# fpthink/3D-WSIS

Measured on AMD Instinct MI355X. Metric: scenes/sec fwd+bwd ScanNet 2cm (~150k voxels) @1/8 GPU; HBM GB/s vs roofline, higher is better.
Workload: dtype f32; 1 GPU; C2: 1 synthetic ScanNet-shaped scene on 1 GPU, 2 cm voxels, fwd+bwd+AdamW step (SubMConv3d UNet 32..160 + ECC GNN + edge affinity + MultiTaskLoss); per-batch segment CSRs / edge graph and all rulebooks are rebuilt inside every step; active_voxels=153685, points=199790, superpoints=2289, edges=20054, scenes_per_gpu=1, global_batch=1, parallelism=scene-sharded dp1

## Files before the change

3d-wsis_amd/csrc/gru.hip:

```cpp
#include <algorithm>
#include <cstdlib>

#include "common.h"

using namespace wsis;

namespace {

constexpr int GC = 32;
constexpr int G3 = 96;
constexpr int GRU_WAVES = 4;
constexpr int GRU_WF = 8;
constexpr int GRU_P = 2 * G3 * GC + GC * GC + 2 * G3 + GC;

__device__ __forceinline__ float wsum(float v) {
#pragma unroll
  for (int off = 32; off >= 1; off >>= 1) v += __shfl_xor(v, off, 64);
  return v;
}
__device__ __forceinline__ float sigm(float v) { return 1.0f / (1.0f + expf(-v)); }

struct GruLds {
  float WigT[GC][GC + 1];
  float WihT[GC][G3 + 1];
  float WhhT[GC][G3 + 1];
  float Wih[G3][GC];
  float Whh[G3][GC];
  float Wig[GC][GC];
  float row[GRU_WF][4][G3];
};

template <int NT>
__device__ __forceinline__ void gru_load_weights(GruLds& L, const float* Wig, const float* Wih, const float* Whh,
// ... 119 lines not shown
    for (int u = 0; u < U; ++u) acc += v[u];
  }
  for (; j < end; j += 2) acc += m[(int64_t)perm[j] * GC + c];
  acc += __shfl_xor(acc, 32, 64);
  const int cnt = end - beg;
  return acc / (float)(cnt > 0 ? cnt : 1);
}

template <bool MEAN>
__global__ __launch_bounds__(64 * GRU_WF) void gru_fwd_kernel(
    const float* __restrict__ x, const int32_t* __restrict__ perm, const int32_t* __restrict__ off,
    float* __restrict__ x_out, const float* __restrict__ h, const float* __restrict__ Wig,
    const float* __restrict__ big, const float* __restrict__ Wih, const float* __restrict__ Whh,
    const float* __restrict__ bih, const float* __restrict__ bhh, float* __restrict__ hy, int64_t S) {
  extern __shared__ __attribute__((aligned(16))) unsigned char smem[];
  GruLds& L = *reinterpret_cast<GruLds*>(smem);
  gru_load_weights<64 * GRU_WF>(L, Wig, Wih, Whh, false);
  __syncthreads();
  const int lane = threadIdx.x & 63, wave = threadIdx.x >> 6;
  const int64_t nw = (int64_t)gridDim.x * GRU_WF;
  for (int64_t row = (int64_t)blockIdx.x * GRU_WF + wave; row < S; row += nw) {
    float xv;
    if (MEAN) {
      xv = gru_seg_mean(x, perm, off, row, lane);
      if (lane < 32) x_out[row * GC + lane] = xv;
    } else {
      xv = x[row * GC + (lane & 31)];
    }
    const GruRow R = gru_row_fwd(L, wave, lane, xv, h, big, bih, bhh, row);
    if (lane < 32) hy[row * GC + lane] = R.hy;
  }
}

__global__ __launch_bounds__(64 * GRU_WAVES) void gru_bwd_kernel(
    const float* __restrict__ x, const float* __restrict__ h, const float* __restrict__ Wig,
    const float* __restrict__ big, const float* __restrict__ Wih, const float* __restrict__ Whh,
    const float* __restrict__ bih, const float* __restrict__ bhh, const float* __restrict__ dhy,
    const float* __restrict__ dhy2, int64_t dhy2_pitch,
    float* __restrict__ dx, float* __restrict__ dh, float* __restrict__ partial, int64_t S) {
  extern __shared__ __attribute__((aligned(16))) unsigned char smem[];
  GruLds& L = *reinterpret_cast<GruLds*>(smem);
  gru_load_weights<64 * GRU_WAVES>(L, Wig, Wih, Whh, true);
  __syncthreads();
  const int lane = threadIdx.x & 63, wave = threadIdx.x >> 6;
  const int c = lane & 31, hi = lane >> 5;
  const bool two = lane < 32;
  const int64_t nw = (int64_t)gridDim.x * GRU_WAVES;
  float aWih[48], aWhh[48], aWig[16];
#pragma unroll
  for (int t = 0; t < 48; ++t) aWih[t] = aWhh[t] = 0.f;
#pragma unroll
  for (int t = 0; t < 16; ++t) aWig[t] = 0.f;
  float abih1 = 0.f, abih2 = 0.f, abhh1 = 0.f, abhh2 = 0.f, abig = 0.f;
  float* hrow = L.row[wave][0];
  float* xrow = L.row[wave][1];
  float* dgi = L.row[wave][2];
  float* dgh = L.row[wave][3];
  for (int64_t row = (int64_t)blockIdx.x * GRU_WAVES + wave; row < S; row += nw) {
    const GruRow R = gru_row_fwd(L, wave, lane, x[row * GC + c], h, big, bih, bhh, row);
    float g = dhy ? dhy[row * GC + c] : 0.0f;
    if (dhy2) g = dhy ? g + dhy2[row * dhy2_pitch + c] : dhy2[row * dhy2_pitch + c];
    const float dn = g * (1.0f - R.z);
    const float dz = g * (R.h - R.n);
    float dhc = g * R.z;
    const float dn_pre = dn * (1.0f - R.n * R.n);
    const float ghn = R.gh2 + bhh[64 + c];
    const float dr = dn_pre * ghn;
    const float dz_pre = dz * R.z * (1.0f - R.z);
    const float dr_pre = dr * R.r * (1.0f - R.r);
    const float dz_pre_up = __shfl(dz_pre, c, 64);
    const float y_i1 = two ? dr_pre : dz_pre_up;
    const float y_h1 = y_i1;
    const float y_i2 = dn_pre;
    const float y_h2 = dn_pre * R.r;
    abih1 += y_i1;
    abhh1 += y_h1;
    if (two) {
      abih2 += y_i2;
      abhh2 += y_h2;
    }
    const float inv96 = 1.0f / (float)G3;
    const float m1i = wsum(y_i1 + (two ? y_i2 : 0.f)) * inv96;
    const float m2i = wsum(y_i1 * R.gi1 + (two ? y_i2 * R.gi2 : 0.f)) * inv96;
    const float m1h = wsum(y_h1 + (two ? y_h2 : 0.f)) * inv96;
    const float m2h = wsum(y_h1 * R.gh1 + (two ? y_h2 * R.gh2 : 0.f)) * inv96;
    const float dgi1 = (y_i1 - m1i - R.gi1 * m2i) * R.sig_i;
    const float dgi2 = (y_i2 - m1i - R.gi2 * m2i) * R.sig_i;
    const float dgh1 = (y_h1 - m1h - R.gh1 * m2h) * R.sig_h;
    const float dgh2 = (y_h2 - m1h - R.gh2 * m2h) * R.sig_h;
    dgi[lane] = dgi1;
    dgh[lane] = dgh1;
    if (two) {
      dgi[64 + lane] = dgi2;
      dgh[64 + lane] = dgh2;
    }
    float dxin = 0.f, dhh = 0.f;
#pragma unroll
    for (int t = 0; t < 48; ++t) {
      const int o = hi + 2 * t;
      const float gi_o = dgi[o], gh_o = dgh[o];
      dxin += L.Wih[o][c] * gi_o;
      dhh += L.Whh[o][c] * gh_o;
      aWih[t] += gi_o * xrow[c];
      aWhh[t] += gh_o * hrow[c];
    }
    dxin += __shfl_xor(dxin, 32, 64);
    dhh += __shfl_xor(dhh, 32, 64);
    const float dxc = dxin * R.gin;
    const float dgin = dxin * R.x;
    const float dgpre = dgin * R.gin * (1.0f - R.gin);
    abig += dgpre;
    float* dgp = dgi;
    if (lane < 32) dgp[c] = dgpre;
    float dhg = 0.f;
#pragma unroll
    for (int t = 0; t < 16; ++t) {
      const int cc = hi + 2 * t;
      const float gp = dgp[cc];
      dhg += L.Wig[cc][c] * gp;
      aWig[t] += gp * hrow[c];
    }
    dhg += __shfl_xor(dhg, 32, 64);
    dhc += dhh + dhg;
    if (lane < 32) {
      dx[row * GC + c] = dxc;
      dh[row * GC + c] = dhc;
    }
  }
  __syncthreads();
  float* const mine = reinterpret_cast<float*>(smem) + wave * GRU_P;
#pragma unroll
  for (int t = 0; t < 48; ++t) {
    const int o = hi + 2 * t;
    mine[o * GC + c] = aWih[t];
    mine[G3 * GC + o * GC + c] = aWhh[t];
  }
#pragma unroll
  for (int t = 0; t < 16; ++t) mine[2 * G3 * GC + (hi + 2 * t) * GC + c] = aWig[t];
  {
    float* pb = mine + 2 * G3 * GC + GC * GC;
    pb[lane] = abih1;
    pb[G3 + lane] = abhh1;
    if (two) {
      pb[64 + lane] = abih2;
      pb[G3 + 64 + lane] = abhh2;
      pb[2 * G3 + lane] = abig;
    }
  }
  __syncthreads();
  const float* const s0 = reinterpret_cast<const float*>(smem);
  float* p = partial + (int64_t)blockIdx.x * GRU_P;
  for (int f = threadIdx.x; f < GRU_P; f += blockDim.x) {
    float v = s0[f];
#pragma unroll
    for (int w = 1; w < GRU_WAVES; ++w) v += s0[w * GRU_P + f];
    p[f] = v;
  }
}

constexpr int RED_OUT = 32;
constexpr int RED_LANES = 8;

__global__ __launch_bounds__(RED_OUT * RED_LANES) void gru_reduce_kernel(
    const float* __restrict__ partial, int nslab, float* __restrict__ dWih, float* __restrict__ dWhh,
    float* __restrict__ dWig, float* __restrict__ dbih, float* __restrict__ dbhh, float* __restrict__ dbig) {
  __shared__ float part[RED_LANES][RED_OUT];
  const int ox = threadIdx.x % RED_OUT, sy = threadIdx.x / RED_OUT;
  const int i = blockIdx.x * RED_OUT + ox;
  float s = 0.f;
  if (i < GRU_P) {
    int k = sy;
    for (; k + 15 * RED_LANES < nslab; k += 16 * RED_LANES) {
      float t[16];
#pragma unroll
      for (int j = 0; j < 16; ++j) t[j] = partial[(int64_t)(k + j * RED_LANES) * GRU_P + i];
#pragma unroll
      for (int j = 0; j < 16; ++j) s += t[j];
    }
    for (; k < nslab; k += RED_LANES) s += partial[(int64_t)k * GRU_P + i];
  }
  part[sy][ox] = s;
  __syncthreads();
  if (sy != 0 || i >= GRU_P) return;
#pragma unroll
  for (int y = 1; y < RED_LANES; ++y) s += part[y][ox];
  if (i < G3 * GC)
    dWih[i] = s;
  else if (i < 2 * G3 * GC)
    dWhh[i - G3 * GC] = s;
  else if (i < 2 * G3 * GC + GC * GC)
    dWig[i - 2 * G3 * GC] = s;
  else if (i < 2 * G3 * GC + GC * GC + G3)
    dbih[i - (2 * G3 * GC + GC * GC)] = s;
  else if (i < 2 * G3 * GC + GC * GC + 2 * G3)
    dbhh[i - (2 * G3 * GC + GC * GC + G3)] = s;
  else
    dbig[i - (2 * G3 * GC + GC * GC + 2 * G3)] = s;
}

int gru_blocks(int64_t S, int waves = GRU_WAVES, int rows_per_wave = 3) {
  const char* e = getenv("WSIS_GRU_ROWS");
  if (e && waves == GRU_WAVES && atoi(e) > 0) rows_per_wave = atoi(e);
  int64_t b = ceil_div(S, waves * rows_per_wave);
  if (b < 1) b = 1;
  if (b > 256) b = 256;
  return (int)b;
}

}

extern "C" {

int64_t wsis_gru_cell_workspace_bytes(int64_t S) {
  if (S < 0) return -1;
  return (int64_t)gru_blocks(S) * GRU_P * (int64_t)sizeof(float) + 256;
}

static int gru_fwd_impl(const float* d_x, const int32_t* d_perm, const int32_t* d_off, float* d_x_out, const float* d_h,
                        const float* d_Wig, const float* d_big, const float* d_Wih, const float* d_Whh, const float* d_bih,
                        const float* d_bhh, float* d_hy, int64_t S, void* stream) {
  const size_t lds = sizeof(GruLds);
  static bool attr_set = false;
  if (!attr_set) {
    WSIS_HIP_CHECK(hipFuncSetAttribute((const void*)gru_fwd_kernel<false>, hipFuncAttributeMaxDynamicSharedMemorySize, (int)lds));
    WSIS_HIP_CHECK(hipFuncSetAttribute((const void*)gru_fwd_kernel<true>, hipFuncAttributeMaxDynamicSharedMemorySize, (int)lds));
    attr_set = true;
  }
  if (d_perm)
    hipLaunchKernelGGL(gru_fwd_kernel<true>, dim3(gru_blocks(S, GRU_WF, 1)), dim3(64 * GRU_WF), lds, as_stream(stream), d_x,
                       d_perm, d_off, d_x_out, d_h, d_Wig, d_big, d_Wih, d_Whh, d_bih, d_bhh, d_hy, S);
  else
    hipLaunchKernelGGL(gru_fwd_kernel<false>, dim3(gru_blocks(S, GRU_WF, 1)), dim3(64 * GRU_WF), lds, as_stream(stream), d_x,
                       d_perm, d_off, d_x_out, d_h, d_Wig, d_big, d_Wih, d_Whh, d_bih, d_bhh, d_hy, S);
  WSIS_LAUNCH_CHECK();
  return WSIS_OK;
}

int wsis_gru_cell_fwd(const float* d_x, const float* d_h, const float* d_Wig, const float* d_big,
                      const float* d_Wih, const float* d_Whh, const float* d_bih, const float* d_bhh, float* d_hy,
// ... 39 lines not shown
  return WSIS_OK;
}

int wsis_gru_cell_bwd(const float* d_x, const float* d_h, const float* d_Wig, const float* d_big,
                      const float* d_Wih, const float* d_Whh, const float* d_bih, const float* d_bhh,
                      const float* d_dhy, float* d_dx, float* d_dh, float* d_dWig, float* d_dbig, float* d_dWih,
                      float* d_dWhh, float* d_dbih, float* d_dbhh, int64_t S, int32_t C, void* d_ws,
                      int64_t ws_bytes, void* stream) {
  WSIS_REQUIRE(S >= 1 && C == GC, "GRUCellEx kernel supports C == 32, S >= 1");
  WSIS_REQUIRE(d_x && d_h && d_Wig && d_big && d_Wih && d_Whh && d_bih && d_bhh && d_dhy && d_dx && d_dh &&
                   d_dWig && d_dbig && d_dWih && d_dWhh && d_dbih && d_dbhh && d_ws,
               "null pointer");
  WSIS_REQUIRE(ws_bytes >= wsis_gru_cell_workspace_bytes(S), "workspace too small");
  return gru_bwd_impl(d_x, d_h, d_Wig, d_big, d_Wih, d_Whh, d_bih, d_bhh, d_dhy, nullptr, 0, d_dx, d_dh, d_dWig, d_dbig, d_dWih,
                      d_dWhh, d_dbih, d_dbhh, S, 0, gru_blocks(S), d_ws, as_stream(stream));
}

int wsis_gru_cell_bwd_seq(const float* d_x, const float* d_h, const float* d_Wig, const float* d_big,
                          const float* d_Wih, const float* d_Whh, const float* d_bih, const float* d_bhh,
                          const float* d_dhy, const float* d_dhy2, int64_t dhy2_pitch, float* d_dx, float* d_dh, float* d_dWig,
                          float* d_dbig, float* d_dWih, float* d_dWhh, float* d_dbih, float* d_dbhh, int64_t S, int32_t C,
                          int32_t slot, int32_t n_slots, int32_t finish, void* d_ws, int64_t ws_bytes, void* stream) {
  WSIS_REQUIRE(S >= 1 && C == GC, "GRUCellEx kernel supports C == 32, S >= 1");
  WSIS_REQUIRE(n_slots >= 1 && slot >= 0 && slot < n_slots, "bad slot");
  WSIS_REQUIRE(d_x && d_h && d_Wig && d_big && d_Wih && d_Whh && d_bih && d_bhh && (d_dhy || d_dhy2) && d_dx && d_dh && d_ws,
               "null pointer");
  WSIS_REQUIRE(!d_dhy2 || dhy2_pitch >= GC, "pitch of the second gradient");
  WSIS_REQUIRE(!finish || (d_dWig && d_dbig && d_dWih && d_dWhh && d_dbih && d_dbhh), "null pointer");
  WSIS_REQUIRE(ws_bytes >= (wsis_gru_cell_workspace_bytes(S) - 256) * n_slots + 256, "workspace too small");
  return gru_bwd_impl(d_x, d_h, d_Wig, d_big, d_Wih, d_Whh, d_bih, d_bhh, d_dhy, d_dhy2, dhy2_pitch, d_dx, d_dh, d_dWig, d_dbig,
                      d_dWih, d_dWhh, d_dbih, d_dbhh, S, slot, finish ? gru_blocks(S) * n_slots : 0, d_ws, as_stream(stream));
}

}
```

3d-wsis_amd/wsis_native/__init__.py:

```python
import ctypes
import os
from ctypes import c_char_p, c_double, c_float, c_int32, c_int64, c_void_p

_HERE = os.path.dirname(os.path.abspath(__file__))
_PKG = os.path.dirname(_HERE)

_host = None
_hip = None

I32 = c_int32
I64 = c_int64
F32 = c_float
F64 = c_double
P = c_void_p


class WsisError(RuntimeError):
    pass


def _load(name):
    path = os.path.join(_PKG, name)
    if not os.path.exists(path):
        raise WsisError(
# ... 72 lines not shown
    "wsis_bn_stats": (I32, [P, I64, I32, P, P, P, P, F32, P, I64, P]),
    "wsis_bn_apply": (I32, [P, P, P, P, P, F32, I32, P, I64, I32, P]),
    "wsis_bn_apply_lp": (I32, [P, P, P, P, P, F32, I32, P, I32, I64, I32, I32, P]),
    "wsis_bn_bwd": (I32, [P, P, P, P, P, P, F32, I32, I32, P, P, P, P, I64, I32, P, I64, P]),
    "wsis_segment_csr_workspace_bytes": (I64, [I64, I64]),
    "wsis_segment_csr": (I32, [P, I64, I64, P, P, P, I64, P]),
    "wsis_segment_csr_batch_workspace_bytes": (I64, [I64]),
    "wsis_segment_csr_batch": (I32, [I32, P, P, P, P, P, P, I64, P]),
    "wsis_segment_reduce_fwd": (I32, [P, P, P, P, P, I64, I64, I32, I32, P]),
    "wsis_segment_reduce_bwd": (I32, [P, P, P, P, P, I64, I64, I32, I32, P]),
    "wsis_gather_rows": (I32, [P, P, I32, P, I64, I32, P]),
    "wsis_edge_affinity_fwd": (I32, [P, P, P, P, P, P, P, P, F32, P, P, I64, I64, I32, P]),
    "wsis_edge_affinity_bwd": (I32, [P] * 11 + [F32] + [P] * 7 + [I64, I64, I64, I32, P]),
    "wsis_ecc_message_fwd": (I32, [P, P, P, P, P, P, I64, I64, I32, P]),
    "wsis_ecc_message_bwd": (I32, [P, P, P, P, P, P, P, P, P, I64, I64, I32, P]),
    "wsis_ecc_contract_fwd": (I32, [P, P, P, P, P, I64, I64, P]),
    "wsis_ecc_contract_bwd": (I32, [P, P, P, P, P, P, P, I64, I64, P]),
    "wsis_ecc_contract_bwd_acc": (I32, [P, P, P, P, P, P, P, I64, I64, I32, P]),
    "wsis_ecc_contract_bwd_mean": (I32, [P, P, P, P, P, P, P, P, P, I64, I64, I32, P]),
    "wsis_ecc_u_fwd": (I32, [P, P, P, I64, P]),
    "wsis_gru_cell_workspace_bytes": (I64, [I64]),
    "wsis_gru_cell_fwd": (I32, [P] * 9 + [I64, I32, P]),
    "wsis_gru_cell_bwd": (I32, [P] * 17 + [I64, I32, P, I64, P]),
    "wsis_colsum_workspace_bytes": (I64, [I64, I32]),
    "wsis_colsum": (I32, [P, I64, I32, P, P, I64, P, P]),
    "wsis_pos_enc_workspace_bytes": (I64, [I64]),
    "wsis_pos_enc_fwd": (I32, [P, P, P, P, P, P, P, P, I64, P]),
    "wsis_pos_enc_bwd": (I32, [P, P, P, P, P, P, P, P, P, P, P, I64, P, I64, P]),
    "wsis_heads_workspace_bytes": (I64, [I64, I32, I32]),
    "wsis_heads_fwd": (I32, [P, P, I64, F32, F32, I32, P, P, I64, P]),
    "wsis_heads_bwd": (I32, [P, P, I64, I32, P, P, P, I64, P]),
    "wsis_gru_cell_bwd_seq": (I32, [P] * 10 + [I64] + [P] * 8 + [I64, I32, I32, I32, I32, P, I64, P]),
    "wsis_gru_cell_fwd_mean": (I32, [P] * 12 + [I64, I32, P]),
    "wsis_affinity_dense_build": (I32, [P, P, P, I64, P, I64, P]),
    "wsis_affinity_transition": (I32, [P, P, P, P, P, I32, F32, P, I64, P]),
    "wsis_dgemm": (I32, [P, P, P, I64, I64, I64, P]),
    "wsis_affinity_colmax": (I32, [P, P, I32, P, P, I64, P]),
    "wsis_affinity_propagate_sparse_workspace_bytes": (I64, [I64, I32]),
    "wsis_affinity_propagate_sparse": (I32, [P, P, P, P, P, P, P, I32, I32, F32, I32, I64, P, P, I64, P, P, P, I64, P]),
    "wsis_ballquery_workspace_bytes": (I64, [I64]),
    "wsis_ballquery_count": (I32, [P, P, P, I64, I32, F32, P, P, P, I64, P]),
    "wsis_ballquery_fill": (I32, [P, P, P, I64, I32, F32, P, P, I64, P, I64, P]),
    "wsis_cc_same_label": (I32, [P, P, P, I64, P, P, P, P]),
    "wsis_bfs_order": (I32, [P, P, P, P, P, I64, P, P, P, P]),
    "wsis_plane_score_workspace_bytes": (I64, [I64, I32]),
    "wsis_plane_score": (I32, [P, I64, P, I32, F64, P, P, P, I64, P]),
    "wsis_plane_mark": (I32, [P, I64, P, F64, P, P]),
    "wsis_wl_sp_stats": (I32, [P, P, P, I64, I64, P, P, P, P]),
    "wsis_wl_neighbor_source": (I32, [P, I64, P, P, P, P, F64, I64, P, P]),
    "wsis_wl_apply_source": (I32, [P, P, P, P, P, P, I64, I64, P, P, P, P, P]),
    "wsis_wl_scene_assign": (I32, [P, I64, P, P, P, P, P, P, P, P, F64, I64, P, P, P, P, P, P]),
    "wsis_wl_point_labels": (I32, [P, I64, P, P, P, P, P]),
    "wsis_wl_occupancy_workspace_bytes": (I64, [I64]),
    "wsis_wl_occupancy": (I32, [P, P, P, I64, I32, F32, P, P, I64, P]),
    "wsis_wl_instance_size": (I32, [P, P, I64, I32, P, P, P]),
    "wsis_wl_label_stats": (I32, [P, P, P, P, I64, P, I32, P, P]),
    "wsis_sp_state_bytes": (I64, []),
    "wsis_sp_state_init": (I32, [P, P]),
    "wsis_sp_affine": (I32, [P, I32, P, I64, I64, P, F64, P, P, P, P]),
    "wsis_sp_crop_mask": (I32, [P, I64, P, I32, P, P, P, P, I32, P]),
    "wsis_sp_emit_workspace_bytes": (I64, [I64, I64, I64]),
    "wsis_sp_emit": (I32, [P, P, I64, I64, I64, P, P, P, P, P, P, P, P, P, I64, I64] + [P] * 9 + [P, I64, P]),
    "wsis_sp_tables": (I32, [P, I64, I64, P, P, P, P, P, P]),
    "wsis_sp_relabel": (I32, [P, P, I64, P, I64, P, I64, P, P, P, P]),
    "wsis_sp_instance_info": (I32, [P, P, P, I64, I64, P, P, P]),
    "wsis_gp_sp_moments": (I32, [P, P, P, I64, I64, P, P, P, P, P, P, P, P]),
# ... 97 lines not shown


_SYNC = {}


def sync_block(device=None):
    import torch
    dev = torch.cuda.current_device() if device is None else torch.device(device).index
    if dev is None:
        dev = torch.cuda.current_device()
    key = (dev, torch._C._cuda_getCurrentRawStream(dev))
    t = _SYNC.get(key)
    if t is None:
        t = _SYNC[key] = torch.zeros(int(hip().wsis_sync_bytes()), dtype=torch.uint8, device=torch.device("cuda", dev))
    return t


def sync_err_words(device):
    import torch
    dev = torch.device(device)
    return [t.view(torch.int32).view(-1, 1024)[:, 19] for (d, _), t in _SYNC.items() if d == dev.index]


def sync_errors():
    bad = []
    for (dev, st), t in _SYNC.items():
        w = t.view(__import__("torch").int32).view(-1, 1024)[:, 19]
        for i in w.nonzero().flatten().tolist():
            bad.append((dev, st, int(i)))
    return bad


HEADS_MAX = 8


class Heads(ctypes.Structure):
    _fields_ = [("n_heads", c_int32), ("n_lin", c_int32), ("cout", c_int32 * HEADS_MAX)] + \
               [(name, c_void_p * HEADS_MAX) for name in
                ("W1", "b1", "gamma", "beta", "W2", "b2", "running_mean", "running_var", "hidden", "out", "dout",
                 "dW1", "db1", "dgamma", "dbeta", "dW2", "db2")]


def require_cuda(*tensors):
    for t in tensors:
        if t is not None and not t.is_cuda:
            raise WsisError("this operator runs on the MI355X only: got a CPU tensor (there is no CPU fallback)")


def i32x3(v):
    if isinstance(v, int):
        v = (v, v, v)
    v = [int(x) for x in v]
    assert len(v) == 3
    return (c_int32 * 3)(*v)
```

3d-wsis_amd/wsis_ops.py:

```python
import ctypes
import os

import numpy as np
import torch
from torch.autograd import Function

import wsis_native as _n
from torch_scatter import SegmentCSR


def branch_stream(device, i=0):
    if os.environ.get("WSIS_BRANCH", "1") == "0" or device.type != "cuda":
        return None
    from spconv import ops as sp_ops
    return sp_ops._side_stream(device)


class EdgeGraph(object):

    def __init__(self, edge_u, edge_v, num_nodes, num_src=None, csr_u=None, csr_v=None):
        _n.require_cuda(edge_u, edge_v)
        self.eu = edge_u.contiguous().long()
        self.ev = edge_v.contiguous().long()
        self.E = self.eu.numel()
# ... 510 lines not shown
            if own:
                _n.check(lib.wsis_gru_cell_fwd_mean(_n.ptr(m), _n.ptr(csr_src.perm), _n.ptr(csr_src.offsets), _n.ptr(inp),
                                                    _n.ptr(hxs[i]), *[_n.ptr(t) for t in gp], _n.ptr(hxs[i + 1]), S, 32,
                                                    st), "gru_cell_fwd_mean")
            else:
                _n.check(lib.wsis_segment_reduce_fwd(_n.ptr(m), _n.ptr(csr_src.perm), _n.ptr(csr_src.offsets),
                                                     _n.ptr(inp), None, E, S, 32, 1, st), "segment_reduce_fwd")
                _n.check(lib.wsis_gru_cell_fwd(_n.ptr(inp), _n.ptr(hxs[i]), *[_n.ptr(t) for t in gp], _n.ptr(hxs[i + 1]),
                                               S, 32, st), "gru_cell_fwd")
            Us.append(U)
            inps.append(inp)
        ctx.save_for_backward(h, Waug, *gp, hx_all, *inps, *Us)
        ctx.meta = (csr_src, csr_dst, repeats, cat_all)
        return torch.cat(hxs, 1) if cat_all else hxs[-1].clone()

    @staticmethod
    def backward(ctx, dout):
        csr_src, csr_dst, R, cat_all = ctx.meta
        sv = ctx.saved_tensors
        h, Waug, gp = sv[0], sv[1], list(sv[2:8])
        hx_all, inps, Us = sv[8], sv[9:9 + R], sv[9 + R:9 + 2 * R]
        lib = _n.hip()
        st = _n.stream_ptr()
        E = h.shape[0]
        S = hx_all.shape[0] // (R + 1)
        hxs = [hx_all[i * S:(i + 1) * S] for i in range(R + 1)]
        dev = h.device
        dout = dout.contiguous().float()
        d_slices = [dout[:, 32 * i:32 * (i + 1)] for i in range(R + 1)] if cat_all else None
        own = os.environ.get("WSIS_ECC_OWN_GEMM", "1") != "0"
        pitch = dout.shape[1]
        d_carry = None if cat_all else dout
        dh = torch.empty_like(h) if R > 0 else torch.zeros_like(h)
        dgp = [torch.empty_like(t) for t in gp] if R > 0 else [torch.zeros_like(t) for t in gp]
        ws_bytes = (lib.wsis_gru_cell_workspace_bytes(S) - 256) * max(R, 1) + 256
        ws = torch.empty(ws_bytes, dtype=torch.uint8, device=dev)
        dU_all = torch.empty((R * S, Waug.shape[1]), dtype=torch.float32, device=dev)
        WaugT = Waug.t()
        for i in reversed(range(R)):
            d_inp, d_hprev = torch.empty((S, 32), dtype=torch.float32, device=dev), torch.empty((S, 32), dtype=torch.float32,
                                                                                                device=dev)
            if own:
                extra = (dout.data_ptr() + 4 * 32 * (i + 1)) if cat_all else None
            else:
                extra = None
                if cat_all:
                    d_carry = d_slices[i + 1].contiguous() if d_carry is None else d_carry.add_(d_slices[i + 1])
            _n.check(lib.wsis_gru_cell_bwd_seq(_n.ptr(inps[i]), _n.ptr(hxs[i]), *[_n.ptr(t) for t in gp], _n.ptr(d_carry),
                                               extra, pitch, _n.ptr(d_inp), _n.ptr(d_hprev), *[_n.ptr(t) for t in dgp], S,
                                               32, R - 1 - i, R, 1 if i == 0 else 0, _n.ptr(ws), ws_bytes, st),
                     "gru_cell_bwd_seq")
            dU = dU_all[i * S:(i + 1) * S]
            if own:
                _n.check(lib.wsis_ecc_contract_bwd_mean(_n.ptr(h), _n.ptr(Us[i]), _n.ptr(d_inp), _n.ptr(csr_src.index),
                                                        _n.ptr(csr_src.offsets), _n.ptr(csr_dst.perm),
                                                        _n.ptr(csr_dst.offsets), _n.ptr(dU), _n.ptr(dh), S, E,
                                                        0 if i == R - 1 else 1, st), "ecc_contract_bwd_mean")
            else:
                d_m = torch.empty((E, 32), dtype=torch.float32, device=dev)
                _n.check(lib.wsis_segment_reduce_bwd(_n.ptr(d_inp), _n.ptr(csr_src.index), _n.ptr(csr_src.offsets), None,
                                                     _n.ptr(d_m), E, S, 32, 1, st), "segment_reduce_bwd")
                _n.check(lib.wsis_ecc_contract_bwd_acc(_n.ptr(h), _n.ptr(Us[i]), _n.ptr(d_m), _n.ptr(csr_dst.perm),
                                                       _n.ptr(csr_dst.offsets), _n.ptr(dU), _n.ptr(dh), S, E,
                                                       0 if i == R - 1 else 1, st), "ecc_contract_bwd")
            d_carry = d_hprev.addmm_(dU, WaugT)
        if R == 0:
            d_hx = d_slices[0].contiguous() if cat_all else dout
        else:
            d_hx = d_carry.add_(d_slices[0]) if cat_all else d_carry
        dWaug = None
        if ctx.needs_input_grad[2] and R == 0:
            dWaug = torch.zeros_like(Waug)
        elif ctx.needs_input_grad[2]:
            from spconv import ops as sp_ops
            dWaug = sp_ops._dw(hx_all[:R * S], None, None, dU_all, 1, 32, Waug.shape[1]).view(32, Waug.shape[1])
        need = ctx.needs_input_grad
        return (d_hx if need[0] else None, dh if need[1] else None, dWaug,
                *[g if need[3 + j] else None for j, g in enumerate(dgp)], None, None, None, None)


def ecc_gru_loop(hx, h, Waug, cell, csr_src, csr_dst, repeats, cat_all):
    ig = cell._modules["ig"]
    return _EccGruLoop.apply(hx, h, Waug, ig.weight, ig.bias, cell.weight_ih, cell.weight_hh, cell.bias_ih,
                             cell.bias_hh, csr_src, csr_dst, int(repeats), bool(cat_all))



_TALL_MIN_ROWS = int(__import__("os").environ.get("WSIS_TALL_MIN_ROWS", "1024"))


def colsum(x):
    M, C = x.shape
    if not x.is_cuda or C % 4 != 0 or C > 1024 or C < 4 or x.dtype != torch.float32 or not x.is_contiguous():
        return x.sum(0)
    lib = _n.hip()
    ws_bytes = lib.wsis_colsum_workspace_bytes(M, C)
    ws = torch.empty(ws_bytes, dtype=torch.uint8, device=x.device)
    out = torch.empty(C, dtype=torch.float32, device=x.device)
    _n.check(lib.wsis_colsum(_n.ptr(x), M, C, _n.ptr(out), _n.ptr(ws), ws_bytes, _n.ptr(_n.sync_block(x.device)),
                             _n.stream_ptr()), "colsum")
    return out

# ... 382 lines not shown
```

include/wsis_hip.h:

```cpp
#ifndef WSIS_HIP_H_
#define WSIS_HIP_H_

#include <stdint.h>

#ifdef __cplusplus
extern "C" {
#endif

#define WSIS_ABI_VERSION 2

#define WSIS_OK 0
#define WSIS_ERR_ARG (-1)
#define WSIS_ERR_HIP (-2)
#define WSIS_ERR_OVERFLOW (-3)


int wsis_host_version(void);
const char* wsis_host_last_error(void);

int wsis_host_voxelize_idx_map(const int64_t* h_coords, int64_t N, int32_t* h_p2v, int64_t* M,
                               int32_t* max_active);
int wsis_host_voxelize_idx_fill(const int64_t* h_coords, int64_t N, const int32_t* h_p2v, int64_t M,
                                int32_t max_active, int64_t* h_voxel_locs, int32_t* h_v2p);

// ... 246 lines not shown
  const float* b2[WSIS_HEADS_MAX];
  float* running_mean[WSIS_HEADS_MAX];
  float* running_var[WSIS_HEADS_MAX];
  float* hidden[WSIS_HEADS_MAX];
  float* out[WSIS_HEADS_MAX];
  const float* dout[WSIS_HEADS_MAX];
  float* dW1[WSIS_HEADS_MAX];
  float* db1[WSIS_HEADS_MAX];
  float* dgamma[WSIS_HEADS_MAX];
  float* dbeta[WSIS_HEADS_MAX];
  float* dW2[WSIS_HEADS_MAX];
  float* db2[WSIS_HEADS_MAX];
} wsis_heads;
int64_t wsis_heads_workspace_bytes(int64_t S, int32_t n_heads, int32_t n_lin);
int wsis_heads_fwd(const wsis_heads* h, const float* d_x, int64_t S, float eps, float momentum, int32_t training,
                   float* d_saved, void* d_ws, int64_t ws_bytes, void* stream);
int wsis_heads_bwd(const wsis_heads* h, const float* d_x, int64_t S, int32_t training, const float* d_saved, float* d_dx,
                   void* d_ws, int64_t ws_bytes, void* stream);

int64_t wsis_gru_cell_workspace_bytes(int64_t S);
int wsis_gru_cell_fwd(const float* d_x, const float* d_h, const float* d_Wig, const float* d_big,
                      const float* d_Wih, const float* d_Whh, const float* d_bih, const float* d_bhh, float* d_hy,
                      int64_t S, int32_t C, void* stream);
int wsis_gru_cell_bwd(const float* d_x, const float* d_h, const float* d_Wig, const float* d_big,
                      const float* d_Wih, const float* d_Whh, const float* d_bih, const float* d_bhh,
                      const float* d_dhy, float* d_dx, float* d_dh, float* d_dWig, float* d_dbig, float* d_dWih,
                      float* d_dWhh, float* d_dbih, float* d_dbhh, int64_t S, int32_t C, void* d_ws,
                      int64_t ws_bytes, void* stream);
int wsis_gru_cell_bwd_seq(const float* d_x, const float* d_h, const float* d_Wig, const float* d_big,
                          const float* d_Wih, const float* d_Whh, const float* d_bih, const float* d_bhh,
                          const float* d_dhy, const float* d_dhy2, int64_t dhy2_pitch, float* d_dx, float* d_dh, float* d_dWig,
                          float* d_dbig, float* d_dWih, float* d_dWhh, float* d_dbih, float* d_dbhh, int64_t S, int32_t C,
                          int32_t slot, int32_t n_slots, int32_t finish, void* d_ws, int64_t ws_bytes, void* stream);
int wsis_gru_cell_fwd_mean(const float* d_m, const int32_t* d_perm, const int32_t* d_off, float* d_x_out, const float* d_h,
                           const float* d_Wig, const float* d_big, const float* d_Wih, const float* d_Whh, const float* d_bih,
                           const float* d_bhh, float* d_hy, int64_t S, int32_t C, void* stream);

int wsis_affinity_dense_build(const int64_t* d_eu, const int64_t* d_ev, const float* d_aff, int64_t E,
                              double* d_A, int64_t S, void* stream);
int wsis_affinity_transition(const double* d_A, const uint8_t* d_adj, const int32_t* d_pred,
                             const float* d_conf, const int32_t* d_label, int32_t cls, float thr,
                             double* d_T0, int64_t S, void* stream);
int wsis_dgemm(const double* d_A, const double* d_B, double* d_C, int64_t M, int64_t N, int64_t Kd,
               void* stream);
int wsis_affinity_colmax(const double* d_T, const int32_t* d_label, int32_t cls, double* d_scores,
                         int32_t* d_arg, int64_t S, void* stream);
int64_t wsis_affinity_propagate_sparse_workspace_bytes(int64_t S, int32_t n_present);
int wsis_affinity_propagate_sparse(const double* d_A, const uint8_t* d_adj, const int32_t* d_pred, const float* d_conf,
                                   const int32_t* d_label, const int32_t* d_cls_of, const int32_t* d_ci_of_cls,
                                   int32_t n_present, int32_t class_num, float thr, int32_t iterations, int64_t S,
                                   int32_t* d_col, double* d_val, int64_t nnz_cap, double* d_scores, int32_t* d_arg,
                                   void* d_ws, int64_t ws_bytes, void* stream);

int64_t wsis_ballquery_workspace_bytes(int64_t N);
int wsis_ballquery_count(const float* d_xyz, const int32_t* d_batch_idx, const int32_t* d_batch_off,
                         int64_t N, int32_t B, float radius, int32_t* d_start_len, int32_t* d_total,
                         void* d_ws, int64_t ws_bytes, void* stream);
int wsis_ballquery_fill(const float* d_xyz, const int32_t* d_batch_idx, const int32_t* d_batch_off,
                        int64_t N, int32_t B, float radius, const int32_t* d_start_len, int32_t* d_idx,
                        int64_t total, void* d_ws, int64_t ws_bytes, void* stream);

int wsis_cc_same_label(const int32_t* d_sem, const int32_t* d_idx, const int32_t* d_start_len, int64_t N,
                       int32_t* d_parent, int32_t* d_root, int32_t* d_size, void* stream);
int wsis_bfs_order(const int32_t* d_idx, const int32_t* d_start_len, const int32_t* d_sem, const int32_t* d_seeds,
                   const int32_t* d_offsets, int64_t n_clusters, int32_t* d_pos, int32_t* d_stamp,
                   int32_t* d_cluster_idxs, void* stream);
// ... 147 lines not shown
```

Baseline: 117.1 scenes/s.

## Split GRU backward into lean row kernel plus MFMA parameter-gradient reduction

The GRU cell backward no longer accumulates weight gradients in registers per wave. A lean kernel writes the per-row gate gradients and activations to global buffers, and a separate kernel computes all weight and bias gradients for all recurrent steps at once as outer-product sums on MFMA 32x32x2 instructions, followed by the existing slab reduce. This removes the 112-register accumulator pressure and the per-step partial reductions, and allows 8 waves per block. In exchange it adds extra HBM traffic for the G and A buffers (about 416 floats per row) and one more launch.

```diff
diff --git a/3d-wsis_amd/csrc/gru.hip b/3d-wsis_amd/csrc/gru.hip
--- a/3d-wsis_amd/csrc/gru.hip
+++ b/3d-wsis_amd/csrc/gru.hip
@@ -1,4 +1,5 @@
 #include <algorithm>
+#include <cstdint>
 #include <cstdlib>
 
 #include "common.h"
@@ -184,6 +185,119 @@
   }
 }
 
+struct GruAcc {
+  float Wih[48], Whh[48], Wig[16];
+  float bih1, bih2, bhh1, bhh2, big;
+};
+
+constexpr int GRU_GW = WSIS_GRU_LEAN_G;
+constexpr int GRU_AW = WSIS_GRU_LEAN_A;
+static_assert(GRU_GW == 3 * G3 + 2 * GC && GRU_AW == 2 * GC, "row layouts of include/wsis_hip.h");
+
+template <bool LEAN>
+__device__ __forceinline__ void gru_bwd_row(GruLds& L, int wave, int lane, int64_t row, const float* __restrict__ x,
+                                            const float* __restrict__ h, const float* __restrict__ big,
+                                            const float* __restrict__ bih, const float* __restrict__ bhh,
+                                            const float* __restrict__ dhy, const float* __restrict__ dhy2,
+                                            int64_t dhy2_pitch, float* __restrict__ dx, float* __restrict__ dh, GruAcc& acc,
+                                            float* __restrict__ G, float* __restrict__ A) {
+  const int c = lane & 31, hi = lane >> 5;
+  const bool two = lane < 32;
+  float* hrow = L.row[wave][0];
+  float* xrow = L.row[wave][1];
+  float* dgi = L.row[wave][2];
+  float* dgh = L.row[wave][3];
+  const GruRow R = gru_row_fwd(L, wave, lane, x[row * GC + c], h, big, bih, bhh, row);
+  float g = dhy ? dhy[row * GC + c] : 0.0f;
+  if (dhy2) g = dhy ? g + dhy2[row * dhy2_pitch + c] : dhy2[row * dhy2_pitch + c];
+  const float dn = g * (1.0f - R.z);
+  const float dz = g * (R.h - R.n);
+  float dhc = g * R.z;
+  const float dn_pre = dn * (1.0f - R.n * R.n);
+  const float ghn = R.gh2 + bhh[64 + c];
+  const float dr = dn_pre * ghn;
+  const float dz_pre = dz * R.z * (1.0f - R.z);
+  const float dr_pre = dr * R.r * (1.0f - R.r);
+  const float dz_pre_up = __shfl(dz_pre, c, 64);
+  const float y_i1 = two ? dr_pre : dz_pre_up;
+  const float y_h1 = y_i1;
+  const float y_i2 = dn_pre;
+  const float y_h2 = dn_pre * R.r;
+  if (!LEAN) {
+    acc.bih1 += y_i1;
+    acc.bhh1 += y_h1;
+    if (two) {
+      acc.bih2 += y_i2;
+      acc.bhh2 += y_h2;
+    }
+  }
+  const float inv96 = 1.0f / (float)G3;
+  const float m1i = wsum(y_i1 + (two ? y_i2 : 0.f)) * inv96;
+  const float m2i = wsum(y_i1 * R.gi1 + (two ? y_i2 * R.gi2 : 0.f)) * inv96;
+  const float m1h = wsum(y_h1 + (two ? y_h2 : 0.f)) * inv96;
+  const float m2h = wsum(y_h1 * R.gh1 + (two ? y_h2 * R.gh2 : 0.f)) * inv96;
+  const float dgi1 = (y_i1 - m1i - R.gi1 * m2i) * R.sig_i;
+  const float dgi2 = (y_i2 - m1i - R.gi2 * m2i) * R.sig_i;
+  const float dgh1 = (y_h1 - m1h - R.gh1 * m2h) * R.sig_h;
+  const float dgh2 = (y_h2 - m1h - R.gh2 * m2h) * R.sig_h;
+  dgi[lane] = dgi1;
+  dgh[lane] = dgh1;
+  if (two) {
+    dgi[64 + lane] = dgi2;
+    dgh[64 + lane] = dgh2;
+  }
+  if (LEAN) {
+    float* g_row = G + row * GRU_GW;
+    g_row[lane] = dgi1;
+    g_row[G3 + lane] = dgh1;
+    g_row[2 * G3 + GC + lane] = y_i1;
+    if (two) {
+      g_row[64 + lane] = dgi2;
+      g_row[G3 + 64 + lane] = dgh2;
+      g_row[2 * G3 + GC + 64 + lane] = y_i2;
+      g_row[3 * G3 + GC + lane] = y_h2;
+    }
+    A[row * GRU_AW + lane] = two ? R.xin : R.h;
+  }
+  float dxin = 0.f, dhh = 0.f;
+#pragma unroll
+  for (int t = 0; t < 48; ++t) {
+    const int o = hi + 2 * t;
+    const float gi_o = dgi[o], gh_o = dgh[o];
+    dxin += L.Wih[o][c] * gi_o;
+    dhh += L.Whh[o][c] * gh_o;
+    if (!LEAN) {
+      acc.Wih[t] += gi_o * xrow[c];
+      acc.Whh[t] += gh_o * hrow[c];
+    }
+  }
+  dxin += __shfl_xor(dxin, 32, 64);
+  dhh += __shfl_xor(dhh, 32, 64);
+  const float dxc = dxin * R.gin;
+  const float dgin = dxin * R.x;
+  const float dgpre = dgin * R.gin * (1.0f - R.gin);
+  if (!LEAN) acc.big += dgpre;
+  float* dgp = dgi;
+  if (lane < 32) {
+    dgp[c] = dgpre;
+    if (LEAN) G[row * GRU_GW + 2 * G3 + c] = dgpre;
+  }
+  float dhg = 0.f;
+#pragma unroll
+  for (int t = 0; t < 16; ++t) {
+    const int cc = hi + 2 * t;
+    const float gp = dgp[cc];
+    dhg += L.Wig[cc][c] * gp;
+    if (!LEAN) acc.Wig[t] += gp * hrow[c];
+  }
+  dhg += __shfl_xor(dhg, 32, 64);
+  dhc += dhh + dhg;
+  if (lane < 32) {
+    dx[row * GC + c] = dxc;
+    dh[row * GC + c] = dhc;
+  }
+}
+
 __global__ __launch_bounds__(64 * GRU_WAVES) void gru_bwd_kernel(
     const float* __restrict__ x, const float* __restrict__ h, const float* __restrict__ Wig,
     const float* __restrict__ big, const float* __restrict__ Wih, const float* __restrict__ Whh,
@@ -198,105 +312,32 @@
   const int c = lane & 31, hi = lane >> 5;
   const bool two = lane < 32;
   const int64_t nw = (int64_t)gridDim.x * GRU_WAVES;
-  float aWih[48], aWhh[48], aWig[16];
-#pragma unroll
-  for (int t = 0; t < 48; ++t) aWih[t] = aWhh[t] = 0.f;
-#pragma unroll
-  for (int t = 0; t < 16; ++t) aWig[t] = 0.f;
-  float abih1 = 0.f, abih2 = 0.f, abhh1 = 0.f, abhh2 = 0.f, abig = 0.f;
-  float* hrow = L.row[wave][0];
-  float* xrow = L.row[wave][1];
-  float* dgi = L.row[wave][2];
-  float* dgh = L.row[wave][3];
-  for (int64_t row = (int64_t)blockIdx.x * GRU_WAVES + wave; row < S; row += nw) {
-    const GruRow R = gru_row_fwd(L, wave, lane, x[row * GC + c], h, big, bih, bhh, row);
-    float g = dhy ? dhy[row * GC + c] : 0.0f;
-    if (dhy2) g = dhy ? g + dhy2[row * dhy2_pitch + c] : dhy2[row * dhy2_pitch + c];
-    const float dn = g * (1.0f - R.z);
-    const float dz = g * (R.h - R.n);
-    float dhc = g * R.z;
-    const float dn_pre = dn * (1.0f - R.n * R.n);
-    const float ghn = R.gh2 + bhh[64 + c];
-    const float dr = dn_pre * ghn;
-    const float dz_pre = dz * R.z * (1.0f - R.z);
-    const float dr_pre = dr * R.r * (1.0f - R.r);
-    const float dz_pre_up = __shfl(dz_pre, c, 64);
-    const float y_i1 = two ? dr_pre : dz_pre_up;
-    const float y_h1 = y_i1;
-    const float y_i2 = dn_pre;
-    const float y_h2 = dn_pre * R.r;
-    abih1 += y_i1;
-    abhh1 += y_h1;
-    if (two) {
-      abih2 += y_i2;
-      abhh2 += y_h2;
-    }
-    const float inv96 = 1.0f / (float)G3;
-    const float m1i = wsum(y_i1 + (two ? y_i2 : 0.f)) * inv96;
-    const float m2i = wsum(y_i1 * R.gi1 + (two ? y_i2 * R.gi2 : 0.f)) * inv96;
-    const float m1h = wsum(y_h1 + (two ? y_h2 : 0.f)) * inv96;
-    const float m2h = wsum(y_h1 * R.gh1 + (two ? y_h2 * R.gh2 : 0.f)) * inv96;
-    const float dgi1 = (y_i1 - m1i - R.gi1 * m2i) * R.sig_i;
-    const float dgi2 = (y_i2 - m1i - R.gi2 * m2i) * R.sig_i;
-    const float dgh1 = (y_h1 - m1h - R.gh1 * m2h) * R.sig_h;
-    const float dgh2 = (y_h2 - m1h - R.gh2 * m2h) * R.sig_h;
-    dgi[lane] = dgi1;
-    dgh[lane] = dgh1;
-    if (two) {
-      dgi[64 + lane] = dgi2;
-      dgh[64 + lane] = dgh2;
-    }
-    float dxin = 0.f, dhh = 0.f;
-#pragma unroll
-    for (int t = 0; t < 48; ++t) {
-      const int o = hi + 2 * t;
-      const float gi_o = dgi[o], gh_o = dgh[o];
-      dxin += L.Wih[o][c] * gi_o;
-      dhh += L.Whh[o][c] * gh_o;
-      aWih[t] += gi_o * xrow[c];
-      aWhh[t] += gh_o * hrow[c];
-    }
-    dxin += __shfl_xor(dxin, 32, 64);
-    dhh += __shfl_xor(dhh, 32, 64);
-    const float dxc = dxin * R.gin;
-    const float dgin = dxin * R.x;
-    const float dgpre = dgin * R.gin * (1.0f - R.gin);
-    abig += dgpre;
-    float* dgp = dgi;
-    if (lane < 32) dgp[c] = dgpre;
-    float dhg = 0.f;
-#pragma unroll
-    for (int t = 0; t < 16; ++t) {
-      const int cc = hi + 2 * t;
-      const float gp = dgp[cc];
-      dhg += L.Wig[cc][c] * gp;
-      aWig[t] += gp * hrow[c];
-    }
-    dhg += __shfl_xor(dhg, 32, 64);
-    dhc += dhh + dhg;
-    if (lane < 32) {
-      dx[row * GC + c] = dxc;
-      dh[row * GC + c] = dhc;
-    }
-  }
+  GruAcc acc;
+#pragma unroll
+  for (int t = 0; t < 48; ++t) acc.Wih[t] = acc.Whh[t] = 0.f;
+#pragma unroll
+  for (int t = 0; t < 16; ++t) acc.Wig[t] = 0.f;
+  acc.bih1 = acc.bih2 = acc.bhh1 = acc.bhh2 = acc.big = 0.f;
+  for (int64_t row = (int64_t)blockIdx.x * GRU_WAVES + wave; row < S; row += nw)
+    gru_bwd_row<false>(L, wave, lane, row, x, h, big, bih, bhh, dhy, dhy2, dhy2_pitch, dx, dh, acc, nullptr, nullptr);
   __syncthreads();
   float* const mine = reinterpret_cast<float*>(smem) + wave * GRU_P;
 #pragma unroll
   for (int t = 0; t < 48; ++t) {
     const int o = hi + 2 * t;
-    mine[o * GC + c] = aWih[t];
-    mine[G3 * GC + o * GC + c] = aWhh[t];
-  }
-#pragma unroll
-  for (int t = 0; t < 16; ++t) mine[2 * G3 * GC + (hi + 2 * t) * GC + c] = aWig[t];
+    mine[o * GC + c] = acc.Wih[t];
+    mine[G3 * GC + o * GC + c] = acc.Whh[t];
+  }
+#pragma unroll
+  for (int t = 0; t < 16; ++t) mine[2 * G3 * GC + (hi + 2 * t) * GC + c] = acc.Wig[t];
   {
     float* pb = mine + 2 * G3 * GC + GC * GC;
-    pb[lane] = abih1;
-    pb[G3 + lane] = abhh1;
+    pb[lane] = acc.bih1;
+    pb[G3 + lane] = acc.bhh1;
     if (two) {
-      pb[64 + lane] = abih2;
-      pb[G3 + 64 + lane] = abhh2;
-      pb[2 * G3 + lane] = abig;
+      pb[64 + lane] = acc.bih2;
+      pb[G3 + 64 + lane] = acc.bhh2;
+      pb[2 * G3 + lane] = acc.big;
     }
   }
   __syncthreads();
@@ -350,6 +391,92 @@
     dbig[i - (2 * G3 * GC + GC * GC + 2 * G3)] = s;
 }
 
+template <int WAVES>
+__global__ __launch_bounds__(64 * WAVES) void gru_bwd_lean_kernel(
+    const float* __restrict__ x, const float* __restrict__ h, const float* __restrict__ Wig,
+    const float* __restrict__ big, const float* __restrict__ Wih, const float* __restrict__ Whh,
+    const float* __restrict__ bih, const float* __restrict__ bhh, const float* __restrict__ dhy,
+    const float* __restrict__ dhy2, int64_t dhy2_pitch, float* __restrict__ dx, float* __restrict__ dh,
+    float* __restrict__ G, float* __restrict__ A, int64_t S) {
+  static_assert(WAVES <= GRU_WF, "GruLds::row holds GRU_WF waves");
+  extern __shared__ __attribute__((aligned(16))) unsigned char smem[];
+  GruLds& L = *reinterpret_cast<GruLds*>(smem);
+  gru_load_weights<64 * WAVES>(L, Wig, Wih, Whh, true);
+  __syncthreads();
+  const int lane = threadIdx.x & 63, wave = threadIdx.x >> 6;
+  const int64_t nw = (int64_t)gridDim.x * WAVES;
+  GruAcc none;
+  for (int64_t row = (int64_t)blockIdx.x * WAVES + wave; row < S; row += nw)
+    gru_bwd_row<true>(L, wave, lane, row, x, h, big, bih, bhh, dhy, dhy2, dhy2_pitch, dx, dh, none, G, A);
+}
+
+typedef float gru_f32x16 __attribute__((ext_vector_type(16)));
+constexpr int PG_U = 4;
+
+__global__ __launch_bounds__(64) void gru_param_grad_kernel(const float* __restrict__ G, const float* __restrict__ A,
+                                                            int64_t rows, int chunk, float* __restrict__ slabs) {
+  const int lane = threadIdx.x, c = lane & 31, hi = lane >> 5;
+  const int64_t beg = (int64_t)blockIdx.x * chunk;
+  const int64_t end = beg + chunk < rows ? beg + chunk : rows;
+  gru_f32x16 acc[7];
+#pragma unroll
+  for (int k = 0; k < 7; ++k)
+#pragma unroll
+    for (int r = 0; r < 16; ++r) acc[k][r] = 0.f;
+  float sb[5] = {0.f, 0.f, 0.f, 0.f, 0.f};
+  for (int64_t r0 = beg; r0 < end; r0 += 2 * PG_U) {
+    float a[PG_U][7], y[PG_U][4], xin[PG_U], hv[PG_U];
+#pragma unroll
+    for (int u = 0; u < PG_U; ++u) {
+      const int64_t row = r0 + 2 * u + hi;
+      const bool ok = row < end;
+      const float* g = G + (ok ? row : beg) * GRU_GW;
+      const float* ar = A + (ok ? row : beg) * GRU_AW;
+#pragma unroll
+      for (int k = 0; k < 7; ++k) a[u][k] = g[32 * k + c];
+#pragma unroll
+      for (int k = 0; k < 4; ++k) y[u][k] = g[2 * G3 + GC + 32 * k + c];
+      xin[u] = ar[c];
+      hv[u] = ar[GC + c];
+      if (!ok) {
+#pragma unroll
+        for (int k = 0; k < 7; ++k) a[u][k] = 0.f;
+#pragma unroll
+        for (int k = 0; k < 4; ++k) y[u][k] = 0.f;
+        xin[u] = hv[u] = 0.f;
+      }
+    }
+#pragma unroll
+    for (int u = 0; u < PG_U; ++u) {
+#pragma unroll
+      for (int k = 0; k < 3; ++k) acc[k] = __builtin_amdgcn_mfma_f32_32x32x2f32(a[u][k], xin[u], acc[k], 0, 0, 0);
+#pragma unroll
+      for (int k = 3; k < 7; ++k) acc[k] = __builtin_amdgcn_mfma_f32_32x32x2f32(a[u][k], hv[u], acc[k], 0, 0, 0);
+#pragma unroll
+      for (int k = 0; k < 4; ++k) sb[k] += y[u][k];
+      sb[4] += a[u][6];
+    }
+  }
+  float* p = slabs + (int64_t)blockIdx.x * GRU_P;
+#pragma unroll
+  for (int k = 0; k < 7; ++k)
+#pragma unroll
+    for (int r = 0; r < 16; ++r) p[k * GC * GC + ((r & 3) + 8 * (r >> 2) + 4 * hi) * GC + c] = acc[k][r];
+  float tot[5];
+#pragma unroll
+  for (int k = 0; k < 5; ++k) tot[k] = sb[k] + __shfl_xor(sb[k], 32, 64);
+  if (hi == 0) {
+    float* pb = p + 2 * G3 * GC + GC * GC;
+    pb[c] = tot[0];
+    pb[32 + c] = tot[1];
+    pb[64 + c] = tot[2];
+    pb[G3 + c] = tot[0];
+    pb[G3 + 32 + c] = tot[1];
+    pb[G3 + 64 + c] = tot[3];
+    pb[2 * G3 + c] = tot[4];
+  }
+}
+
 int gru_blocks(int64_t S, int waves = GRU_WAVES, int rows_per_wave = 3) {
   const char* e = getenv("WSIS_GRU_ROWS");
   if (e && waves == GRU_WAVES && atoi(e) > 0) rows_per_wave = atoi(e);
@@ -357,6 +484,37 @@
   if (b < 1) b = 1;
   if (b > 256) b = 256;
   return (int)b;
+}
+
+constexpr int GRU_LEAN_CAP = 512;
+int gru_lean_blocks(int64_t S, int waves = GRU_WF, int rows_per_wave = 1, int cap = GRU_LEAN_CAP) {
+  int64_t b = ceil_div(S, waves * rows_per_wave);
+  if (b < 1) b = 1;
+  if (b > cap) b = cap;
+  return (int)b;
+}
+
+int gru_param_chunk(int64_t rows) {
+  int c = 64;
+  while (c < 1024 && rows > (int64_t)c * 512) c *= 2;
+  return c;
+}
+
+template <int WAVES>
+int gru_lean_launch(int nb, const float* d_x, const float* d_h, const float* d_Wig, const float* d_big, const float* d_Wih,
+                    const float* d_Whh, const float* d_bih, const float* d_bhh, const float* d_dhy, const float* d_dhy2,
+                    int64_t dhy2_pitch, float* d_dx, float* d_dh, float* d_G, float* d_A, int64_t S, hipStream_t st) {
+  const size_t lds = sizeof(GruLds);
+  static bool attr_set = false;
+  if (!attr_set) {
+    WSIS_HIP_CHECK(hipFuncSetAttribute((const void*)gru_bwd_lean_kernel<WAVES>, hipFuncAttributeMaxDynamicSharedMemorySize,
+                                       (int)lds));
+    attr_set = true;
+  }
+  hipLaunchKernelGGL(gru_bwd_lean_kernel<WAVES>, dim3(nb), dim3(64 * WAVES), lds, st, d_x, d_h, d_Wig, d_big, d_Wih, d_Whh,
+                     d_bih, d_bhh, d_dhy, d_dhy2, dhy2_pitch, d_dx, d_dh, d_G, d_A, S);
+  WSIS_LAUNCH_CHECK();
+  return WSIS_OK;
 }
 
 }
@@ -462,4 +620,40 @@
                       d_dWih, d_dWhh, d_dbih, d_dbhh, S, slot, finish ? gru_blocks(S) * n_slots : 0, d_ws, as_stream(stream));
 }
 
-}
+int wsis_gru_cell_bwd_lean(const float* d_x, const float* d_h, const float* d_Wig, const float* d_big, const float* d_Wih,
+                           const float* d_Whh, const float* d_bih, const float* d_bhh, const float* d_dhy,
+                           const float* d_dhy2, int64_t dhy2_pitch, float* d_dx, float* d_dh, float* d_G, float* d_A,
+                           int64_t S, int32_t C, void* stream) {
+  WSIS_REQUIRE(S >= 1 && C == GC, "GRUCellEx kernel supports C == 32, S >= 1");
+  WSIS_REQUIRE(d_x && d_h && d_Wig && d_big && d_Wih && d_Whh && d_bih && d_bhh && (d_dhy || d_dhy2) && d_dx && d_dh &&
+                   d_G && d_A,
+               "null pointer");
+  WSIS_REQUIRE(!d_dhy2 || dhy2_pitch >= GC, "pitch of the second gradient");
+  return gru_lean_launch<GRU_WF>(gru_lean_blocks(S), d_x, d_h, d_Wig, d_big, d_Wih, d_Whh, d_bih, d_bhh, d_dhy, d_dhy2,
+                                 dhy2_pitch, d_dx, d_dh, d_G, d_A, S, as_stream(stream));
+}
+
+int64_t wsis_gru_param_grads_workspace_bytes(int64_t rows) {
+  if (rows < 0) return -1;
+  return ceil_div(std::max<int64_t>(rows, 1), gru_param_chunk(rows)) * GRU_P * (int64_t)sizeof(float) + 256;
+}
+
+int wsis_gru_param_grads(const float* d_G, const float* d_A, int64_t rows, float* d_dWig, float* d_dbig, float* d_dWih,
+                         float* d_dWhh, float* d_dbih, float* d_dbhh, void* d_ws, int64_t ws_bytes, void* stream) {
+  WSIS_REQUIRE(rows >= 1, "at least one row");
+  WSIS_REQUIRE(d_G && d_A && d_dWig && d_dbig && d_dWih && d_dWhh && d_dbih && d_dbhh && d_ws, "null pointer");
+  WSIS_REQUIRE(ws_bytes >= wsis_gru_param_grads_workspace_bytes(rows), "workspace too small");
+  const int chunk = gru_param_chunk(rows);
+  const int64_t nslab = ceil_div(rows, chunk);
+  WSIS_REQUIRE(nslab <= INT32_MAX, "too many rows");
+  hipStream_t st = as_stream(stream);
+  float* slabs = static_cast<float*>(d_ws);
+  hipLaunchKernelGGL(gru_param_grad_kernel, dim3((unsigned)nslab), dim3(64), 0, st, d_G, d_A, rows, chunk, slabs);
+  WSIS_LAUNCH_CHECK();
+  hipLaunchKernelGGL(gru_reduce_kernel, dim3((GRU_P + RED_OUT - 1) / RED_OUT), dim3(RED_OUT * RED_LANES), 0, st, slabs,
+                     (int)nslab, d_dWih, d_dWhh, d_dWig, d_dbih, d_dbhh, d_dbig);
+  WSIS_LAUNCH_CHECK();
+  return WSIS_OK;
+}
+
+}
diff --git a/3d-wsis_amd/wsis_native/__init__.py b/3d-wsis_amd/wsis_native/__init__.py
--- a/3d-wsis_amd/wsis_native/__init__.py
+++ b/3d-wsis_amd/wsis_native/__init__.py
@@ -128,6 +128,9 @@
     "wsis_heads_bwd": (I32, [P, P, I64, I32, P, P, P, I64, P]),
     "wsis_gru_cell_bwd_seq": (I32, [P] * 10 + [I64] + [P] * 8 + [I64, I32, I32, I32, I32, P, I64, P]),
     "wsis_gru_cell_fwd_mean": (I32, [P] * 12 + [I64, I32, P]),
+    "wsis_gru_cell_bwd_lean": (I32, [P] * 10 + [I64] + [P] * 4 + [I64, I32, P]),
+    "wsis_gru_param_grads_workspace_bytes": (I64, [I64]),
+    "wsis_gru_param_grads": (I32, [P, P, I64] + [P] * 6 + [P, I64, P]),
     "wsis_affinity_dense_build": (I32, [P, P, P, I64, P, I64, P]),
     "wsis_affinity_transition": (I32, [P, P, P, P, P, I32, F32, P, I64, P]),
     "wsis_dgemm": (I32, [P, P, P, I64, I64, I64, P]),
@@ -291,6 +294,7 @@
 
 
 HEADS_MAX = 8
+GRU_LEAN_G, GRU_LEAN_A = 352, 64
 
 
 class Heads(ctypes.Structure):
diff --git a/3d-wsis_amd/wsis_ops.py b/3d-wsis_amd/wsis_ops.py
--- a/3d-wsis_amd/wsis_ops.py
+++ b/3d-wsis_amd/wsis_ops.py
@@ -566,8 +566,14 @@
         pitch = dout.shape[1]
         d_carry = None if cat_all else dout
         dh = torch.empty_like(h) if R > 0 else torch.zeros_like(h)
+        lean = R > 0 and S > 0 and os.environ.get("WSIS_GRU_LEAN", "1") != "0"
         dgp = [torch.empty_like(t) for t in gp] if R > 0 else [torch.zeros_like(t) for t in gp]
-        ws_bytes = (lib.wsis_gru_cell_workspace_bytes(S) - 256) * max(R, 1) + 256
+        if lean:
+            G_all = torch.empty((R * S, _n.GRU_LEAN_G), dtype=torch.float32, device=dev)
+            A_all = torch.empty((R * S, _n.GRU_LEAN_A), dtype=torch.float32, device=dev)
+            ws_bytes = lib.wsis_gru_param_grads_workspace_bytes(R * S)
+        else:
+            ws_bytes = (lib.wsis_gru_cell_workspace_bytes(S) - 256) * max(R, 1) + 256
         ws = torch.empty(ws_bytes, dtype=torch.uint8, device=dev)
         dU_all = torch.empty((R * S, Waug.shape[1]), dtype=torch.float32, device=dev)
         WaugT = Waug.t()
@@ -580,10 +586,16 @@
                 extra = None
                 if cat_all:
                     d_carry = d_slices[i + 1].contiguous() if d_carry is None else d_carry.add_(d_slices[i + 1])
-            _n.check(lib.wsis_gru_cell_bwd_seq(_n.ptr(inps[i]), _n.ptr(hxs[i]), *[_n.ptr(t) for t in gp], _n.ptr(d_carry),
-                                               extra, pitch, _n.ptr(d_inp), _n.ptr(d_hprev), *[_n.ptr(t) for t in dgp], S,
-                                               32, R - 1 - i, R, 1 if i == 0 else 0, _n.ptr(ws), ws_bytes, st),
-                     "gru_cell_bwd_seq")
+            if lean:
+                _n.check(lib.wsis_gru_cell_bwd_lean(_n.ptr(inps[i]), _n.ptr(hxs[i]), *[_n.ptr(t) for t in gp],
+                                                    _n.ptr(d_carry), extra, pitch, _n.ptr(d_inp), _n.ptr(d_hprev),
+                                                    _n.ptr(G_all[i * S:(i + 1) * S]), _n.ptr(A_all[i * S:(i + 1) * S]), S,
+                                                    32, st), "gru_cell_bwd_lean")
+            else:
+                _n.check(lib.wsis_gru_cell_bwd_seq(_n.ptr(inps[i]), _n.ptr(hxs[i]), *[_n.ptr(t) for t in gp],
+                                                   _n.ptr(d_carry), extra, pitch, _n.ptr(d_inp), _n.ptr(d_hprev),
+                                                   *[_n.ptr(t) for t in dgp], S, 32, R - 1 - i, R, 1 if i == 0 else 0,
+                                                   _n.ptr(ws), ws_bytes, st), "gru_cell_bwd_seq")
             dU = dU_all[i * S:(i + 1) * S]
             if own:
                 _n.check(lib.wsis_ecc_contract_bwd_mean(_n.ptr(h), _n.ptr(Us[i]), _n.ptr(d_inp), _n.ptr(csr_src.index),
@@ -602,6 +614,9 @@
             d_hx = d_slices[0].contiguous() if cat_all else dout
         else:
             d_hx = d_carry.add_(d_slices[0]) if cat_all else d_carry
+        if lean:
+            _n.check(lib.wsis_gru_param_grads(_n.ptr(G_all), _n.ptr(A_all), R * S, *[_n.ptr(t) for t in dgp], _n.ptr(ws),
+                                              ws_bytes, st), "gru_param_grads")
         dWaug = None
         if ctx.needs_input_grad[2] and R == 0:
             dWaug = torch.zeros_like(Waug)
diff --git a/include/wsis_hip.h b/include/wsis_hip.h
--- a/include/wsis_hip.h
+++ b/include/wsis_hip.h
@@ -302,6 +302,15 @@
                           const float* d_dhy, const float* d_dhy2, int64_t dhy2_pitch, float* d_dx, float* d_dh, float* d_dWig,
                           float* d_dbig, float* d_dWih, float* d_dWhh, float* d_dbih, float* d_dbhh, int64_t S, int32_t C,
                           int32_t slot, int32_t n_slots, int32_t finish, void* d_ws, int64_t ws_bytes, void* stream);
+#define WSIS_GRU_LEAN_G 352
+#define WSIS_GRU_LEAN_A 64
+int wsis_gru_cell_bwd_lean(const float* d_x, const float* d_h, const float* d_Wig, const float* d_big, const float* d_Wih,
+                           const float* d_Whh, const float* d_bih, const float* d_bhh, const float* d_dhy,
+                           const float* d_dhy2, int64_t dhy2_pitch, float* d_dx, float* d_dh, float* d_G, float* d_A,
+                           int64_t S, int32_t C, void* stream);
+int64_t wsis_gru_param_grads_workspace_bytes(int64_t rows);
+int wsis_gru_param_grads(const float* d_G, const float* d_A, int64_t rows, float* d_dWig, float* d_dbig, float* d_dWih,
+                         float* d_dWhh, float* d_dbih, float* d_dbhh, void* d_ws, int64_t ws_bytes, void* stream);
 int wsis_gru_cell_fwd_mean(const float* d_m, const int32_t* d_perm, const int32_t* d_off, float* d_x_out, const float* d_h,
                            const float* d_Wig, const float* d_big, const float* d_Wih, const float* d_Whh, const float* d_bih,
                            const float* d_bhh, float* d_hy, int64_t S, int32_t C, void* stream);
```

Result: slower. 113.8 scenes/s (-2.8%).
